# microsoft/M3P

Measured on AMD Instinct MI355X. Metric: pre-train samples/sec (whole node), 12L/768d seq=128+36, higher is better.
Workload: dtype bf16; 1 GPU; cfg2: 12L/768d/12h, 36 regions + 128 tokens, V=250002, 19 MLM targets/seq + ITM BCE, dropout 0.10, adam_inverse_sqrt + clip 5; per_gpu_batch=256, global_batch=256, seq_len=164, parallelism=dp1, prewarm_steps=36

## Files before the change

### m3p_amd/csrc/gemm.hip

```cpp
#include <mutex>
#include <type_traits>
#include "common.hpp"
#include "../../include/m3p_hip.h"
#include <hip/amd_detail/amd_hip_unsafe_atomics.h>

static int g_variant = 1;
extern "C" void m3p_debug_set_variant(int v) { g_variant = (v == 2 || v == 6) ? v : 1; }

namespace {

constexpr int BK = 64;
constexpr int ROWB = BK * 2;

#define M3P_DSR(dst, addr, off) asm volatile("ds_read_b128 %0, %1 offset:" #off : "=v"(dst) : "v"(addr))
#define M3P_TR(dst, addr, off) asm volatile("ds_read_b64_tr_b16 %0, %1 offset:" #off : "=v"(dst) : "v"(addr))
#define M3P_WAIT_LGKM(N) do { __builtin_amdgcn_sched_barrier(0); asm volatile("s_waitcnt lgkmcnt(" #N ")" ::: "memory"); __builtin_amdgcn_sched_barrier(0); } while (0)
#define M3P_WAIT_VM(N) do { __builtin_amdgcn_sched_barrier(0); asm volatile("s_waitcnt vmcnt(" #N ")" ::: "memory"); __builtin_amdgcn_sched_barrier(0); } while (0)
#define M3P_BAR() do { __builtin_amdgcn_s_barrier(); asm volatile("" ::: "memory"); __builtin_amdgcn_sched_barrier(0); } while (0)

__device__ __forceinline__ int xcd_slot(int nwg) {
  const int per_xcd = nwg >> 3;
  return (blockIdx.x & 7) * per_xcd + (blockIdx.x >> 3);
}
__device__ __forceinline__ int strip_width(int tiles_n, int from, int width) {
// ... 543 lines not shown
    if (O8) w8[j] = (O8 == 2) ? pack8<true>(v, scale8, *amax) : pack8<false>(v, scale8, *amax);
  }
  if (O8) piece8_write(r8, w8, lane);
  bf16* Cp = C + (size_t)mrow0 * ldc + nw + sch * 8;
  if (O8) {
    const uint32_t la = lds_addr(r1), l8 = lds_addr(r8);
    const int row8 = lane >> 2, c8 = lane & 3;
    u32x4_lds Ra, Rb, R8;
    lds_r128(la + ep_off<true>(srow, sch * 16), Ra);
    lds_r128(la + ep_off<true>(8 + srow, sch * 16), Rb);
    lds_r128(l8 + row8 * 64 + (c8 << 4), R8);
    asm volatile("s_waitcnt lgkmcnt(0)" : "+v"(Ra), "+v"(Rb), "+v"(R8));
    st16p<true>(Cp + (size_t)srow * ldc, u32x4{Ra[0], Ra[1], Ra[2], Ra[3]});
    st16p<true>(Cp + (size_t)(8 + srow) * ldc, u32x4{Rb[2], Rb[3], Rb[0], Rb[1]});
    st16p<true>(o8 + (size_t)(mrow0 + row8) * ld8 + nw + ((c8 ^ ((row8 >> 1) & 3)) << 4), u32x4{R8[0], R8[1], R8[2], R8[3]});
    return;
  }
  u32x4 R2[2];
#pragma unroll
  for (int it = 0; it < 2; ++it) {
    const int row = it * 8 + srow;
    R2[it] = flip_halves(*reinterpret_cast<const u32x4*>(r1 + ep_off<true>(row, sch * 16)), it & 1);
  }
#pragma unroll
  for (int it = 0; it < 2; ++it) st16p<true>(Cp + (size_t)(it * 8 + srow) * ldc, R2[it]);
  if (O8) piece8_store(o8, ld8, mrow0, nw, r8, lane);
}

__device__ __forceinline__ void epilogue_half_lse(bf16* __restrict__ C, int ldc, float2* __restrict__ stats, int V, int mrow0, int nw,
                                                  char* r1, const f32x4 (&rows0)[4], const f32x4 (&rows1)[4],
                                                  const f32x4 (&biasv)[4], int lane, bool edge) {
  constexpr float kLog2e = 1.4426950408889634f;
  const int fr = lane & 15, fg = lane >> 4;
  const int srow = lane >> 3, sch = lane & 7;
#pragma unroll
  for (int ii = 0; ii < 2; ++ii) {
    f32x4 x[4];
#pragma unroll
    for (int j = 0; j < 4; ++j) {
      x[j] = (ii ? rows1[j] : rows0[j]) + biasv[j];
      const bf16x4 xb = bf16x4{(bf16)x[j][0], (bf16)x[j][1], (bf16)x[j][2], (bf16)x[j][3]};
      *reinterpret_cast<bf16x4*>(r1 + ep_off8<true>(ii * 16 + fr, (j * 16 + fg * 4) * 2)) = xb;
#pragma unroll
      for (int r = 0; r < 4; ++r) x[j][r] = (float)xb[r];
    }
    if (edge) {
#pragma unroll
      for (int j = 0; j < 4; ++j)
#pragma unroll
        for (int r = 0; r < 4; ++r)
          if (nw + j * 16 + fg * 4 + r >= V) x[j][r] = -INFINITY;
    }
    f32x4 m4 = x[0];
#pragma unroll
    for (int j = 1; j < 4; ++j)
#pragma unroll
      for (int r = 0; r < 4; ++r) m4[r] = fmaxf(m4[r], x[j][r]);
    float m = fmaxf(fmaxf(m4[0], m4[1]), fmaxf(m4[2], m4[3]));
    m = fmaxf(m, __shfl_xor(m, 16, 64));
    m = fmaxf(m, __shfl_xor(m, 32, 64));
    const float mb = (m == -INFINITY) ? 0.f : m * kLog2e;
    f32x4 s4 = f32x4{0.f, 0.f, 0.f, 0.f};
#pragma unroll
    for (int j = 0; j < 4; ++j) {
      const f32x4 a = x[j] * kLog2e - mb;
#pragma unroll
      for (int r = 0; r < 4; ++r) s4[r] += __builtin_amdgcn_exp2f(a[r]);
    }
    float sm = (s4[0] + s4[1]) + (s4[2] + s4[3]);
    sm += __shfl_xor(sm, 16, 64);
    sm += __shfl_xor(sm, 32, 64);
    if (fg == 0) stats[mrow0 + ii * 16 + fr] = float2{m, sm};
  }
  bf16* Cp = C + (size_t)mrow0 * ldc + nw + sch * 8;
#pragma unroll
  for (int it = 0; it < 4; ++it) {
    const int row = it * 8 + srow;
    st16p<true>(Cp + (size_t)row * ldc, flip_halves(*reinterpret_cast<const u32x4*>(r1 + ep_off<true>(row, sch * 16)), it & 1));
  }
}

constexpr int M3P_EPI_BIAS_EXP = 11;
struct CeRowRef { float c; int32_t y; };
__device__ __forceinline__ void epilogue_half_exp(bf16* __restrict__ C, int ldc, float* __restrict__ stats, const CeRowRef* __restrict__ ref,
                                                  int V, int mrow0, int nw, char* r1, const f32x4 (&rows0)[4], const f32x4 (&rows1)[4],
                                                  const f32x4 (&biasv)[4], int lane, bool edge) {
  constexpr float kLog2e = 1.4426950408889634f;
  const int fr = lane & 15, fg = lane >> 4;
  const int srow = lane >> 3, sch = lane & 7;
  const float2 rf[2] = {*reinterpret_cast<const float2*>(ref + mrow0 + fr), *reinterpret_cast<const float2*>(ref + mrow0 + 16 + fr)};
#pragma unroll
  for (int ii = 0; ii < 2; ++ii) {
    const float cb = rf[ii].x * kLog2e;
    const int tc = __builtin_bit_cast(int, rf[ii].y) - nw - fg * 4;
    f32x4 x[4];
#pragma unroll
    for (int j = 0; j < 4; ++j) {
      const f32x4 a = ((ii ? rows1[j] : rows0[j]) + biasv[j]) * kLog2e - cb;
#pragma unroll
      for (int r = 0; r < 4; ++r) x[j][r] = __builtin_amdgcn_exp2f(a[r]);
    }
    if (edge) {
#pragma unroll
      for (int j = 0; j < 4; ++j)
#pragma unroll
        for (int r = 0; r < 4; ++r)
          if (nw + j * 16 + fg * 4 + r >= V) x[j][r] = 0.f;
    }
    if (__any((unsigned)(tc + fg * 4) < 64u)) {
#pragma unroll
      for (int j = 0; j < 4; ++j)
#pragma unroll
        for (int r = 0; r < 4; ++r)
          if (j * 16 + r == tc) x[j][r] = 0.f;
    }
    f32x4 s4 = f32x4{0.f, 0.f, 0.f, 0.f};
#pragma unroll
    for (int j = 0; j < 4; ++j) {
      const bf16x4 xb = bf16x4{(bf16)x[j][0], (bf16)x[j][1], (bf16)x[j][2], (bf16)x[j][3]};
      *reinterpret_cast<bf16x4*>(r1 + ep_off8<true>(ii * 16 + fr, (j * 16 + fg * 4) * 2)) = xb;
#pragma unroll
      for (int r = 0; r < 4; ++r) s4[r] += (float)xb[r];
    }
    float sm = (s4[0] + s4[1]) + (s4[2] + s4[3]);
    sm += __shfl_xor(sm, 16, 64);
    sm += __shfl_xor(sm, 32, 64);
    if (fg == 0) stats[mrow0 + ii * 16 + fr] = sm;
  }
  bf16* Cp = C + (size_t)mrow0 * ldc + nw + sch * 8;
#pragma unroll
  for (int it = 0; it < 4; ++it) {
    const int row = it * 8 + srow;
    st16p<true>(Cp + (size_t)row * ldc, flip_halves(*reinterpret_cast<const u32x4*>(r1 + ep_off<true>(row, sch * 16)), it & 1));
  }
}

constexpr int GQ_TAB_LO = 0x3A00, GQ_TAB_HI = 0x4100, GQ_TAB_N = GQ_TAB_HI - GQ_TAB_LO;
constexpr int GQ_TAB_BYTES = GQ_TAB_N * 4;
__device__ __forceinline__ void geluq_table_fill(uint32_t* tab, int tid, int nthreads) {
  for (int i = tid; i < GQ_TAB_N; i += nthreads) {
    const float xm = __builtin_bit_cast(float, ((uint32_t)(GQ_TAB_LO + i) << 16) | 0x8000u);
    const float tail = 0.5f * erfcf(xm * 0.70710678118654752440f);
    const float gd = (1.0f - tail) + xm * 0.39894228040143267794f * __expf(-0.5f * xm * xm);
    tab[i] = (__builtin_bit_cast(uint32_t, tail) & 0xFFFFFF00u) | gelu_grad_code(gd);
  }
}
__device__ __forceinline__ void lds_r32(uint32_t a, uint32_t& v) { asm volatile("ds_read_b32 %0, %1" : "=v"(v) : "v"(a)); }
template <int O8 = 0>
__device__ __forceinline__ void epilogue_piece_geluq_lut(bf16* __restrict__ C, int ldc, uint8_t* __restrict__ qout, int mrow0, int nw,
                                                         char* r1, const f32x4 (&rows)[4], int lane, uint32_t tab_off,
                                                         uint8_t* __restrict__ o8 = nullptr, int ld8 = 0, float scale8 = 1.f, float* amax = nullptr,
                                                         char* r8 = nullptr) {
  const int fr = lane & 15, fg = lane >> 4;
  const int srow = lane >> 3, sch = lane & 7;
  uint32_t w8[4];
  uint32_t w[4][4];
#pragma unroll
  for (int j = 0; j < 4; ++j)
#pragma unroll
    for (int r = 0; r < 4; ++r) {
      const float xf = rows[j][r];
      const uint32_t xb = __builtin_bit_cast(uint32_t, xf);
      const uint32_t mag = __builtin_amdgcn_ubfe(xb, 16, 15);
      const uint32_t idx = min(max(mag, (uint32_t)GQ_TAB_LO), (uint32_t)(GQ_TAB_HI - 1));
      lds_r32((idx << 2) + tab_off, w[j][r]);
    }
  asm volatile("s_waitcnt lgkmcnt(0)" : "+v"(w[0][0]), "+v"(w[0][1]), "+v"(w[0][2]), "+v"(w[0][3]), "+v"(w[1][0]), "+v"(w[1][1]), "+v"(w[1][2]), "+v"(w[1][3]),
                                        "+v"(w[2][0]), "+v"(w[2][1]), "+v"(w[2][2]), "+v"(w[2][3]), "+v"(w[3][0]), "+v"(w[3][1]), "+v"(w[3][2]), "+v"(w[3][3]));
  const uint32_t la = lds_addr(r1);
  u32x4 code;
#pragma unroll
  for (int j = 0; j < 4; ++j) {
    f32x4 hv;
    float xs[4];
#pragma unroll
    for (int r = 0; r < 4; ++r) {
      xs[r] = rows[j][r];
      float mx;
      asm("v_max_f32 %0, 0, %1" : "=v"(mx) : "v"(xs[r]));
      asm("v_fma_f32 %0, -|%1|, %2, %3" : "=v"(hv[r]) : "v"(xs[r]), "v"(w[j][r]), "v"(mx));
    }
    const uint32_t x0 = __builtin_bit_cast(uint32_t, xs[0]), x1 = __builtin_bit_cast(uint32_t, xs[1]);
    const uint32_t x2 = __builtin_bit_cast(uint32_t, xs[2]), x3 = __builtin_bit_cast(uint32_t, xs[3]);
    const uint32_t blo = __builtin_amdgcn_perm(w[j][1], w[j][0], 0x0c0c0400u), bhi = __builtin_amdgcn_perm(w[j][3], w[j][2], 0x04000c0cu);
    const uint32_t slo = __builtin_amdgcn_perm(x1, x0, 0x0c0c0b09u), shi = __builtin_amdgcn_perm(x3, x2, 0x0b090c0cu);
    code[j] = (blo | bhi) ^ (slo | shi);
    lds_w64(la + ep_off8<true>(fr, (j * 16 + fg * 4) * 2), bf16x4{(bf16)hv[0], (bf16)hv[1], (bf16)hv[2], (bf16)hv[3]});
    if (O8) w8[j] = pack8<false>(hv, scale8, *amax);
  }
  st16p<true>(qout + lane * 16, code);
  if (O8) piece8_write(r8, w8, lane);
  u32x4 R[2];
  u32x4_lds R8;
  lds_r128(la + ep_off<true>(srow, sch * 16), R[0]);
  lds_r128(la + ep_off<true>(8 + srow, sch * 16), R[1]);
  const int row8 = lane >> 2, c8 = lane & 3;
  if (O8) {
    lds_r128(lds_addr(r8) + row8 * 64 + (c8 << 4), R8);
    asm volatile("s_waitcnt lgkmcnt(0)" : "+v"(R[0]), "+v"(R[1]), "+v"(R8));
  } else {
    asm volatile("s_waitcnt lgkmcnt(0)" : "+v"(R[0]), "+v"(R[1]));
  }
  bf16* Cp = C + (size_t)mrow0 * ldc + nw + sch * 8;
  st16p<true>(Cp + (size_t)srow * ldc, R[0]);
  st16p<true>(Cp + (size_t)(8 + srow) * ldc, flip_halves(R[1], true));
  if (O8) st16p<true>(o8 + (size_t)(mrow0 + row8) * ld8 + nw + ((c8 ^ ((row8 >> 1) & 3)) << 4), u32x4{R8[0], R8[1], R8[2], R8[3]});
}


template <int EPI>
// ... 152 lines not shown
        u32x4 auxt0[4], auxt1[4];
        load_aux_rows_issue<EPI>(ep, mw, nw, lane, auxt0);
        load_aux_rows_issue<EPI>(ep, mw + 32, nw, lane, auxt1);
        auto do_half = [&](const int hf, const u32x4 (&auxt)[4]) {
          f32x4 rows[2][4];
#pragma unroll
          for (int ii = 0; ii < 2; ++ii)
#pragma unroll
            for (int j = 0; j < 4; ++j) rows[ii][j] = acc[2 * hf + ii][j];
          f32x4 biasv[4];
          bf16x4 auxv[2][4];
          load_bias4<EPI>(ep, nw, lane, biasv);
          load_aux_rows_finish<EPI>(lane, r1, auxt, auxv);
          epilogue_half<EPI>(ep, C, ldc, N, mw + 32 * hf, nw, r1, rows, biasv, auxv, lane, csum, gtab);
        };
        do_half(0, auxt0);
        do_half(1, auxt1);
      } else {
#pragma unroll
        for (int i = 0; i < 4; ++i)
#pragma unroll
          for (int j = 0; j < 4; ++j)
            epilogue_store<EPI>(ep, C, ldc, M, N, mw + i * 16 + fr, nw + j * 16 + fg * 4, acc[i][j], csum[j]);
      }
#pragma unroll
      for (int i = 0; i < 4; ++i)
#pragma unroll
        for (int j = 0; j < 4; ++j) acc[i][j] = f32x4{0.f, 0.f, 0.f, 0.f};
      if (step + 1 < total) {
        M3P_WAIT_LGKM(0);
        __builtin_amdgcn_s_barrier();
        asm volatile("" ::: "memory");
      }
    }
    cur = nxt;
  }
  if ((EPI == M3P_EPI_DGELU || EPI == M3P_EPI_MUL) && ep.colsum && csum_nw >= 0) flush_csum();
}


template <class T>
__device__ __forceinline__ const T* uniform_ptr(const T* p) {
  const uint64_t v = reinterpret_cast<uint64_t>(p);
  const uint32_t lo = __builtin_amdgcn_readfirstlane((uint32_t)v), hi = __builtin_amdgcn_readfirstlane((uint32_t)(v >> 32));
  return reinterpret_cast<const T*>(((uint64_t)hi << 32) | lo);
}

template <int EPI, bool DYN = false, bool O8 = false>
__global__ __launch_bounds__(512)
void gemm_nt_w8_kernel(const bf16* __restrict__ A, int lda, const bf16* __restrict__ W, int ldw,
                       bf16* __restrict__ C, int ldc, int M, int N, int K, M3PEpilogue ep,
                       int tiles_m, int tiles_n, int* __restrict__ tile_ctr) {
  constexpr int BM = 256, BN = 256, NWAVES = 8;
  constexpr int A_BYTES = BM * ROWB, STAGE = (BM + BN) * ROWB;
  extern __shared__ __attribute__((aligned(16))) char smem[];

  const int tid = threadIdx.x, lane = tid & 63;
  const int wid = __builtin_amdgcn_readfirstlane(tid >> 6);
  const int ntiles = tiles_m * tiles_n;
  const int strip_w = strip_width(tiles_n, 9, 4);
  auto split_tile = [&](int t, int& tm, int& tn) {
    const int strip = t / (tiles_m * strip_w);
    const int rem = t - strip * tiles_m * strip_w;
    const int bn = min(strip_w, tiles_n - strip * strip_w);
    tm = rem / bn;
    tn = strip * strip_w + (rem - tm * bn);
  };
  const int nwg = gridDim.x;
  const int per_xcd = nwg >> 3;
  const int xcd = blockIdx.x & 7;
  const int slot = xcd_slot(nwg);
  if (slot >= ntiles) return;
  const int nk = K / BK;
  constexpr bool dyn = DYN;
  auto tile_of = [&](int q) { return q * nwg + slot; };
  const int my_tiles = (ntiles - slot + nwg - 1) / nwg;
  const int total = my_tiles * nk;
  int t_ld = slot, t_cmp = slot, t_next = -1;
  int pop_state = 0;
  unsigned popped = 0;
  constexpr bool kMulE = (EPI == M3P_EPI_DGELU || EPI == M3P_EPI_MUL || EPI == M3P_EPI_MULQ);
  constexpr bool kAuxE = (EPI == M3P_EPI_BIAS_DROP_RES || EPI == M3P_EPI_RES || kMulE);
  constexpr bool kGqLut = (EPI == M3P_EPI_BIAS_GELUQ);
  constexpr int kTabBytes = (EPI == M3P_EPI_DGELU) ? GELU_TAB_N * (int)sizeof(float) : (kGqLut ? GQ_TAB_BYTES : 0);
  float* gtab = (EPI == M3P_EPI_DGELU) ? reinterpret_cast<float*>(smem + 2 * STAGE) : nullptr;
  if (EPI == M3P_EPI_DGELU) gelu_grad_table_fill(gtab, tid, 512);
  if (kGqLut) geluq_table_fill(reinterpret_cast<uint32_t*>(smem + 2 * STAGE), tid, 512);
  int* const mbox = reinterpret_cast<int*>(smem + 2 * STAGE + kTabBytes);

  const int sr = lane >> 3, sc = (lane & 7) ^ sr;
  int l_kt = 0, l_q = 0;
  bool l_alive = true;
  __amdgpu_buffer_rsrc_t a_rsrc, w_rsrc;
  auto set_load_tile = [&](int t) {
    int tm, tn;
    split_tile(t, tm, tn);
    const bf16* a_src = A + (size_t)(tm * BM + wid * 32) * lda;
    const bf16* w_src = W + (size_t)(tn * BN + wid * 32) * ldw;
    a_rsrc = __builtin_amdgcn_make_buffer_rsrc(const_cast<bf16*>(uniform_ptr(a_src)), 0, 0xffffffff, 0x00020000);
    w_rsrc = __builtin_amdgcn_make_buffer_rsrc(const_cast<bf16*>(uniform_ptr(w_src)), 0, 0xffffffff, 0x00020000);
  };
  const uint32_t a_lane = (uint32_t)(sr * lda + sc * 8) * 2u, w_lane = (uint32_t)(sr * ldw + sc * 8) * 2u;
  auto issue_load = [&](int s, int piece) {
    char* sa = smem + s * STAGE;
    const int k0 = l_kt * BK;
    const int pc = piece & 3;
    char* base = sa + (piece < 4 ? 0 : A_BYTES) + wid * 4096;
    const uint32_t soff = __builtin_amdgcn_readfirstlane((uint32_t)k0 * 2u + (uint32_t)pc * (uint32_t)((piece < 4 ? lda : ldw) * 16) - (uint32_t)pc * 1024u);
#define W8_LDB(IMM) __builtin_amdgcn_raw_ptr_buffer_load_lds(piece < 4 ? a_rsrc : w_rsrc, LDS_PTR(base), 16, piece < 4 ? a_lane : w_lane, soff, IMM, 0)
    switch (pc) {
      case 0: W8_LDB(0); break;
      case 1: W8_LDB(1024); break;
      case 2: W8_LDB(2048); break;
      default: W8_LDB(3072); break;
    }
#undef W8_LDB
  };
  auto load_done = [&]() {
    if constexpr (!dyn) {
      if (++l_kt == nk) { l_kt = 0; ++l_q; if (l_q < my_tiles) set_load_tile(tile_of(l_q)); }
    } else {
      ++l_kt;
      if (l_kt == 3) {
        pop_state = 1;
        if (wid == 0 && lane == 0) popped = __hip_atomic_fetch_add(reinterpret_cast<unsigned*>(tile_ctr) + xcd, 1u, __ATOMIC_RELAXED, __HIP_MEMORY_SCOPE_AGENT);
      }
      if (l_kt == nk) {
        l_kt = 0;
        t_ld = t_next;
        t_next = -1;
        if (t_ld >= 0) set_load_tile(t_ld); else l_alive = false;
      }
    }
  };
  auto stage_next = [&](int s) {
#pragma unroll
    for (int pc = 0; pc < 8; ++pc) issue_load(s, pc);
    load_done();
  };

  const int wm = wid >> 2, wn = wid & 3;
  const int fr = lane & 15, fg = lane >> 4;
  const uint32_t lds0 = (uint32_t)(uintptr_t)(__attribute__((address_space(3))) char*)smem;
  uint32_t a_addr[2], b_addr[2];
#pragma unroll
  for (int ks = 0; ks < 2; ++ks) {
    const int ch = ((fg + 4 * ks) ^ (fr & 7)) * 16;
    a_addr[ks] = lds0 + (wm * 128 + fr) * ROWB + ch;
    b_addr[ks] = lds0 + A_BYTES + (wn * 64 + fr) * ROWB + ch;
  }
  auto read_w = [&](uint32_t ba, bf16x8 (&wf)[4]) {
    M3P_DSR(wf[0], ba, 0); M3P_DSR(wf[1], ba, 2048); M3P_DSR(wf[2], ba, 4096); M3P_DSR(wf[3], ba, 6144);
  };
  auto read_a_lo = [&](uint32_t aa, bf16x8 (&af)[4]) {
    M3P_DSR(af[0], aa, 0); M3P_DSR(af[1], aa, 2048); M3P_DSR(af[2], aa, 4096); M3P_DSR(af[3], aa, 6144);
  };
  auto read_a_hi = [&](uint32_t aa, bf16x8 (&af)[4]) {
    M3P_DSR(af[0], aa, 8192); M3P_DSR(af[1], aa, 10240); M3P_DSR(af[2], aa, 12288); M3P_DSR(af[3], aa, 14336);
  };

  f32x4 acc[8][4];
#pragma unroll
  for (int i = 0; i < 8; ++i)
#pragma unroll
    for (int j = 0; j < 4; ++j) acc[i][j] = f32x4{0.f, 0.f, 0.f, 0.f};
  if constexpr (kGqLut) {
    int tm0, tn0;
    split_tile(slot, tm0, tn0);
    const float* bp = ep.bias + tn0 * BN + wn * 64 + fg * 4;
#pragma unroll
    for (int j = 0; j < 4; ++j) {
      const f32x4 b = *reinterpret_cast<const f32x4*>(bp + j * 16);
#pragma unroll
      for (int i = 0; i < 8; ++i) acc[i][j] = b;
    }
  }
  auto mfma_q = [&](auto half_c, const bf16x8 (&af)[4], const bf16x8 (&wf)[4]) {
    constexpr int I0 = 4 * decltype(half_c)::value;
    __builtin_amdgcn_s_setprio(1);
#pragma unroll
    for (int i = 0; i < 4; ++i)
#pragma unroll
      for (int j = 0; j < 4; ++j)
        acc[I0 + i][j] = __builtin_amdgcn_mfma_f32_16x16x32_bf16(wf[j], af[i], acc[I0 + i][j], 0, 0, 0);
    __builtin_amdgcn_s_setprio(0);
  };
  using H0 = std::integral_constant<int, 0>;
  using H1 = std::integral_constant<int, 1>;

  set_load_tile(slot);
  stage_next(0);
#define W8_H1 (dyn ? h1d : (step + 1 < total))
#define W8_MORE2 (dyn ? l_alive : more2)
  bool h1d = l_alive;
  if (dyn ? h1d : (total > 1)) {
    stage_next(1);
    asm volatile("s_waitcnt vmcnt(8)" ::: "memory");
  } else {
    asm volatile("s_waitcnt vmcnt(0)" ::: "memory");
  }
  __builtin_amdgcn_s_barrier();
  asm volatile("" ::: "memory");

  bf16x8 fa0[4], fa1[4], fw0[4], fw1[4];
  read_w(b_addr[0], fw0);
  read_a_lo(a_addr[0], fa0);
  M3P_WAIT_LGKM(0);
  int c_kt = 0, c_q = 0;
  const bool io_aligned = ((ldc & 7) == 0) && (((uintptr_t)C & 15) == 0) &&
                          (!(EPI == M3P_EPI_BIAS_GELU) || (((ep.ld_out2 & 7) == 0) && (((uintptr_t)ep.out2 & 15) == 0))) &&
                          (!ep.bias || (((uintptr_t)ep.bias & 15) == 0)) &&
                          (!ep.aux || (((ep.ld_aux & 7) == 0) && (((uintptr_t)ep.aux & 15) == 0)));
  f32x4 csum[4];
#pragma unroll
  for (int j = 0; j < 4; ++j) csum[j] = f32x4{0.f, 0.f, 0.f, 0.f};
  int csum_nw = -1;
  auto flush_csum = [&]() {
#pragma unroll
    for (int j = 0; j < 4; ++j)
#pragma unroll
      for (int r = 0; r < 4; ++r) {
        float sfl = csum[j][r];
        sfl += __shfl_xor(sfl, 1, 64); sfl += __shfl_xor(sfl, 2, 64);
        sfl += __shfl_xor(sfl, 4, 64); sfl += __shfl_xor(sfl, 8, 64);
        const int n = csum_nw + j * 16 + fg * 4 + r;
        if (fr == 0 && n < N) unsafeAtomicAdd(ep.colsum + n, sfl);
        csum[j][r] = 0.f;
      }
  };
  float amax_run = 0.f;
  if constexpr (O8 && EPI == M3P_EPI_MULQ) reinterpret_cast<float*>(smem + 2 * STAGE + 8 * 2048)[tid] = 0.f;
  bool spread_pending = false;
  for (int step = 0; dyn || step < total; ++step) {
    const int cur = step & 1, nxt = cur ^ 1;
    const bool last_kt = (c_kt + 1 == nk);
    const bool more2 = dyn ? false : (step + 2 < total);
    const uint32_t so = cur * STAGE;
    const bool pend = spread_pending;
    if (pend) { issue_load(nxt, 3); issue_load(nxt, 4); issue_load(nxt, 5); }
    read_a_hi(a_addr[0] + so, fa1);
    __builtin_amdgcn_sched_barrier(0);
    mfma_q(H0{}, fa0, fw0);
    M3P_WAIT_LGKM(0);
    if (pend) { issue_load(nxt, 6); issue_load(nxt, 7); }
    read_w(b_addr[1] + so, fw1);
    read_a_lo(a_addr[1] + so, fa0);
    __builtin_amdgcn_sched_barrier(0);
    mfma_q(H1{}, fa1, fw0);
    if (pend) { load_done(); spread_pending = false; }
    M3P_WAIT_LGKM(0);
    read_a_hi(a_addr[1] + so, fa1);
    __builtin_amdgcn_sched_barrier(0);
    mfma_q(H0{}, fa0, fw1);
    M3P_WAIT_LGKM(0);
    asm volatile("s_waitcnt vmcnt(0)" ::: "memory");
    __builtin_amdgcn_s_barrier();
    asm volatile("" ::: "memory");
    __builtin_amdgcn_sched_barrier(0);
    if (dyn && pop_state) {
      if (pop_state == 1) {
        if (wid == 0 && lane == 0) {
          const int p = per_xcd + (int)popped, q = p / per_xcd;
          const int t = q * nwg + xcd * per_xcd + (p - q * per_xcd);
          *mbox = (t < ntiles) ? t : -1;
        }
        pop_state = 2;
      } else {
        t_next = __builtin_amdgcn_readfirstlane(*mbox);
        pop_state = 0;
      }
      __builtin_amdgcn_sched_barrier(0);
    }
    const bool req = W8_MORE2 && (!last_kt || !kAuxE);
    if (req) {
      issue_load(cur, 0); issue_load(cur, 1); issue_load(cur, 2);
      spread_pending = true;
    }
    if (W8_H1 && !last_kt) {
      read_w(b_addr[0] + nxt * STAGE, fw0);
      read_a_lo(a_addr[0] + nxt * STAGE, fa0);
    }
    __builtin_amdgcn_sched_barrier(0);
    mfma_q(H1{}, fa1, fw1);
    M3P_WAIT_LGKM(0);

    if (++c_kt == nk) {
      c_kt = 0;
      const int t = dyn ? t_cmp : tile_of(c_q);
      if (dyn) t_cmp = t_ld; else ++c_q;
      int tm, tn;
      split_tile(t, tm, tn);
      const int m0 = tm * BM, n0 = tn * BN;
      const int mw = m0 + wm * 128, nw = n0 + wn * 64;
      if (kMulE && ep.colsum && csum_nw != nw) {
        if (csum_nw >= 0) flush_csum();
        csum_nw = nw;
      }
      const bool fast = io_aligned && (m0 + BM <= M) && (n0 + BN <= N);
      if constexpr (EPI == M3P_EPI_BIAS_LSE || EPI == M3P_EPI_BIAS_EXP) {
        if (fast) {
          char* r1 = smem + 2 * STAGE + wid * 4096;
          f32x4 biasv[4];
#pragma unroll
          for (int j = 0; j < 4; ++j) biasv[j] = *reinterpret_cast<const f32x4*>(ep.bias + nw + j * 16 + (lane >> 4) * 4);
          const int V = ep.ld_out2;
          const bool edge = (nw + 64 > V);
          if constexpr (EPI == M3P_EPI_BIAS_EXP) {
            float* st = reinterpret_cast<float*>(ep.out2) + (size_t)(tn * 4 + wn) * M;
            const CeRowRef* ref = reinterpret_cast<const CeRowRef*>(ep.row_ref);
#pragma unroll
            for (int hf = 0; hf < 4; ++hf) {
              epilogue_half_exp(C, ldc, st, ref, V, mw + 32 * hf, nw, r1, acc[2 * hf], acc[2 * hf + 1], biasv, lane, edge);
              __builtin_amdgcn_sched_barrier(0);
            }
          } else {
            float2* st = reinterpret_cast<float2*>(ep.out2) + (size_t)(tn * 4 + wn) * M;
#pragma unroll
            for (int hf = 0; hf < 4; ++hf) {
              epilogue_half_lse(C, ldc, st, V, mw + 32 * hf, nw, r1, acc[2 * hf], acc[2 * hf + 1], biasv, lane, edge);
              __builtin_amdgcn_sched_barrier(0);
            }
          }
        }
      } else if constexpr (kGqLut) {
        f32x4 bnext[4];
        {
          const bool more_tiles = dyn ? (t_cmp >= 0) : (c_q < my_tiles);
          int tm2 = tm, tn2 = tn;
          if (more_tiles) split_tile(dyn ? t_cmp : tile_of(c_q), tm2, tn2);
          const float* bp = ep.bias + tn2 * BN + wn * 64 + fg * 4;
#pragma unroll
          for (int j = 0; j < 4; ++j) bnext[j] = *reinterpret_cast<const f32x4*>(bp + j * 16);
        }
        {
          char* r1 = smem + 2 * STAGE + kTabBytes + wid * 2048;
          const uint32_t tab_off = lds0 + 2 * STAGE - 4 * GQ_TAB_LO;
          uint8_t* qo = reinterpret_cast<uint8_t*>(ep.out2) + gq_block_offset(tm, tn, tiles_n, wid, 0);
          if constexpr (O8) {
            const float sc8 = ep.scale8 ? *ep.scale8 : 1.f;
#pragma unroll
            for (int hp = 0; hp < 8; ++hp) {
              epilogue_piece_geluq_lut<1>(C, ldc, qo + 1024 * hp, mw + 16 * hp, nw, r1, acc[hp], lane, tab_off,
                                          reinterpret_cast<uint8_t*>(ep.out8), ep.ld_out8, sc8, &amax_run,
                                          smem + 2 * STAGE + kTabBytes + 8 * 2048 + wid * 1024);
              __builtin_amdgcn_sched_barrier(0);
            }
          } else {
#pragma unroll
            for (int hp = 0; hp < 8; ++hp) {
              epilogue_piece_geluq_lut(C, ldc, qo + 1024 * hp, mw + 16 * hp, nw, r1, acc[hp], lane, tab_off);
              __builtin_amdgcn_sched_barrier(0);
            }
          }
        }
#pragma unroll
        for (int i = 0; i < 8; ++i)
#pragma unroll
          for (int j = 0; j < 4; ++j) acc[i][j] = bnext[j];
      } else if constexpr (EPI == M3P_EPI_MULQ) {
        if (fast) {
          const uint8_t* qp = reinterpret_cast<const uint8_t*>(ep.aux) + gq_block_offset(tm, tn, tiles_n, wid, 0) + lane * 16;
          char* r1 = smem + 2 * STAGE + wid * 2048;
#define MQ_LD(off) (*reinterpret_cast<const u32x4*>(qp + (off)))
          u32x4 qa = MQ_LD(0), qb = MQ_LD(1024);
          __builtin_amdgcn_sched_barrier(0);
          if (W8_MORE2) { issue_load(cur, 0); issue_load(cur, 1); issue_load(cur, 2); spread_pending = true; }
          __builtin_amdgcn_sched_barrier(0);
          if constexpr (O8) {
            const float sc8 = ep.scale8 ? *ep.scale8 : 1.f;
            uint8_t* o8 = reinterpret_cast<uint8_t*>(ep.out8);
            float* amax_slot = reinterpret_cast<float*>(smem + 2 * STAGE + 8 * 2048) + tid;
            float amax_t = *amax_slot;
#pragma unroll
            for (int hp = 0; hp < 8; ++hp) {
              u32x4 qc = qb;
              if (hp + 2 < 8) qc = MQ_LD((hp + 2) * 1024);
              char* r8 = smem + 2 * STAGE + 8 * 2048 + 2048 + wid * 1024;
              epilogue_pieceq<2>(C, ldc, mw + 16 * hp, nw, r1, acc[hp], qa, lane, csum, o8, ep.ld_out8, sc8, &amax_t, r8);
              __builtin_amdgcn_sched_barrier(0);
              qa = qb; qb = qc;
            }
            *amax_slot = amax_t;
          } else {
#pragma unroll
          for (int hp = 0; hp < 8; hp += 2) {
            u32x4 qc = qa, qd = qb;
            if (hp + 2 < 8) qc = MQ_LD((hp + 2) * 1024);
            epilogue_pieceq(C, ldc, mw + 16 * hp, nw, r1, acc[hp], qa, lane, csum);
            __builtin_amdgcn_sched_barrier(0);
            if (hp + 3 < 8) qd = MQ_LD((hp + 3) * 1024);
            epilogue_pieceq(C, ldc, mw + 16 * (hp + 1), nw, r1, acc[hp + 1], qb, lane, csum);
            __builtin_amdgcn_sched_barrier(0);
            qa = qc; qb = qd;
          }
          }
#undef MQ_LD
        }
      } else if (fast && kMulE) {
        char* r1 = smem + 2 * STAGE + kTabBytes + wid * 2048;
        u32x4 ta[2], tb[2];
        aux16_issue(ep, mw, nw, lane, ta);
        __builtin_amdgcn_sched_barrier(0);
        if (W8_MORE2) { issue_load(cur, 0); issue_load(cur, 1); issue_load(cur, 2); spread_pending = true; }
        __builtin_amdgcn_sched_barrier(0);
#pragma unroll
        for (int hp = 0; hp < 8; hp += 2) {
          aux16_issue(ep, mw + 16 * (hp + 1), nw, lane, tb);
          epilogue_piece16<EPI>(ep, C, ldc, mw + 16 * hp, nw, r1, acc[hp], ta, lane, csum, gtab);
          __builtin_amdgcn_sched_barrier(0);
          if (hp + 2 < 8) aux16_issue(ep, mw + 16 * (hp + 2), nw, lane, ta);
          epilogue_piece16<EPI>(ep, C, ldc, mw + 16 * (hp + 1), nw, r1, acc[hp + 1], tb, lane, csum, gtab);
          __builtin_amdgcn_sched_barrier(0);
        }
      } else if (fast) {
        char* r1 = smem + 2 * STAGE + wid * 4096;
        f32x4 biasv[4];
        load_bias4<EPI>(ep, nw, lane, biasv);
        u32x4 aux0[4];
        if (kAuxE) {
          load_aux_rows_issue<EPI>(ep, mw, nw, lane, aux0);
          __builtin_amdgcn_sched_barrier(0);
          if (W8_MORE2) { issue_load(cur, 0); issue_load(cur, 1); issue_load(cur, 2); spread_pending = true; }
          __builtin_amdgcn_sched_barrier(0);
        }
#pragma unroll
        for (int hf = 0; hf < 4; ++hf) {
          f32x4 rows[2][4];
#pragma unroll
          for (int ii = 0; ii < 2; ++ii)
#pragma unroll
            for (int j = 0; j < 4; ++j) rows[ii][j] = acc[2 * hf + ii][j];
          bf16x4 auxv[2][4];
          if (kAuxE && hf == 0) load_aux_rows_finish<EPI, true>(lane, r1, aux0, auxv);
          else load_aux_rows<EPI, true>(ep, mw + 32 * hf, nw, lane, r1, auxv);
          epilogue_half<EPI, true>(ep, C, ldc, N, mw + 32 * hf, nw, r1, rows, biasv, auxv, lane, csum, gtab);
          __builtin_amdgcn_sched_barrier(0);
        }
      } else {
        if (kAuxE && W8_MORE2) { issue_load(cur, 0); issue_load(cur, 1); issue_load(cur, 2); spread_pending = true; }
#pragma unroll
        for (int i = 0; i < 8; ++i)
#pragma unroll
          for (int j = 0; j < 4; ++j)
            epilogue_store<EPI>(ep, C, ldc, M, N, mw + i * 16 + fr, nw + j * 16 + fg * 4, acc[i][j], csum[j]);
      }
      if constexpr (!kGqLut) {
#pragma unroll
        for (int i = 0; i < 8; ++i)
#pragma unroll
          for (int j = 0; j < 4; ++j) acc[i][j] = f32x4{0.f, 0.f, 0.f, 0.f};
      }
      if (W8_H1) {
        read_w(b_addr[0] + nxt * STAGE, fw0);
        read_a_lo(a_addr[0] + nxt * STAGE, fa0);
        M3P_WAIT_LGKM(0);
      }
    }
    if (dyn) {
      if (!h1d) break;
      h1d = l_alive;
    }
  }
  if (kMulE && ep.colsum && csum_nw >= 0) flush_csum();
  if constexpr (O8 && (EPI == M3P_EPI_BIAS_GELUQ || EPI == M3P_EPI_MULQ)) {
    if (ep.amax8) {
      float* wmax = reinterpret_cast<float*>(smem + 2 * STAGE + kTabBytes);
      if constexpr (EPI == M3P_EPI_MULQ) amax_run = reinterpret_cast<float*>(smem + 2 * STAGE + 8 * 2048)[tid];
      const float mxw = wave_max(amax_run);
      __syncthreads();
      if (lane == 0) wmax[wid] = mxw;
      __syncthreads();
      if (tid == 0) {
        float mx = wmax[0];
#pragma unroll
        for (int w = 1; w < NWAVES; ++w) mx = fmaxf(mx, wmax[w]);
        unsigned int* slot = reinterpret_cast<unsigned int*>(ep.amax8);
        if (__float_as_uint(mx) > __builtin_nontemporal_load(slot)) atomicMax(slot, __float_as_uint(mx));
      }
    }
  }
#undef W8_H1
#undef W8_MORE2
}

typedef __attribute__((ext_vector_type(8))) int i32x8;
typedef __attribute__((ext_vector_type(4))) int i32x4;
template <int EPI, bool A_BF8>
__global__ __launch_bounds__(512)
void gemm_nt_w8f8_kernel(const uint8_t* __restrict__ A, int lda, const uint8_t* __restrict__ W, int ldw,
                         bf16* __restrict__ C, int ldc, int M, int N, int K, M3PEpilogue ep,
                         int tiles_m, int tiles_n) {
  constexpr int BM = 256, BN = 256, NWAVES = 8, BK8 = 128;
  constexpr int A_BYTES = BM * ROWB, STAGE = (BM + BN) * ROWB;
  extern __shared__ __attribute__((aligned(16))) char smem[];

  const int tid = threadIdx.x, lane = tid & 63;
  const int wid = __builtin_amdgcn_readfirstlane(tid >> 6);
  const int ntiles = tiles_m * tiles_n;
  const int strip_w = strip_width(tiles_n, 12, 4);
  const int nwg = gridDim.x;
  const int slot = xcd_slot(nwg);
  auto tile_of = [&](int q) { return q * nwg + slot; };
  const int my_tiles = (ntiles > slot) ? (ntiles - slot + nwg - 1) / nwg : 0;
  if (my_tiles == 0) return;
  constexpr bool kMulE = (EPI == M3P_EPI_DGELU || EPI == M3P_EPI_MUL);
  constexpr bool kAuxE = (EPI == M3P_EPI_BIAS_DROP_RES || EPI == M3P_EPI_RES || kMulE);
  constexpr bool kGqLut = (EPI == M3P_EPI_BIAS_GELUQ);
  constexpr int kTabBytes = (EPI == M3P_EPI_DGELU) ? GELU_TAB_N * (int)sizeof(float) : (kGqLut ? GQ_TAB_BYTES : 0);
  float* gtab = (EPI == M3P_EPI_DGELU) ? reinterpret_cast<float*>(smem + 2 * STAGE) : nullptr;
  if (EPI == M3P_EPI_DGELU) gelu_grad_table_fill(gtab, tid, 512);
  if (kGqLut) geluq_table_fill(reinterpret_cast<uint32_t*>(smem + 2 * STAGE), tid, 512);
  const int nk = K / BK8;
  const int total = my_tiles * nk;
  const float dsc = (ep.descale_a ? *ep.descale_a : 1.f) * (ep.descale_b ? *ep.descale_b : 1.f);

  const int sr = lane >> 3, sc = (lane & 7) ^ sr;
  const uint8_t* a_src;
  const uint8_t* w_src;
  const size_t a_step = (size_t)64 * lda, w_step = (size_t)64 * ldw;
  int l_q = 0, l_kt = 0;
  auto set_load_tile = [&](int q) {
    int tm, tn;
    split_tile(tile_of(q), tiles_m, tiles_n, strip_w, tm, tn);
    a_src = A + (size_t)(tm * BM + wid * 8 + sr) * lda + sc * 16;
    w_src = W + (size_t)(tn * BN + wid * 8 + sr) * ldw + sc * 16;
  };
  auto issue_load = [&](int s, int piece) {
    char* sa = smem + s * STAGE;
    const int k0 = l_kt * BK8;
// ... 541 lines not shown
    return M3P_KERN_NT_W4;
  if (M >= 1024) return M3P_KERN_NT_RING;
  return M3P_KERN_NT_128;
}

template <int EPI>
int launch_nt(const bf16* A, int lda, const bf16* W, int ldw, bf16* C, int ldc, int M, int N, int K,
              const M3PEpilogue& ep, hipStream_t st) {
  int want_queue = 0;
  const int plan = nt_plan(EPI, M, N, K, &want_queue);
  if (plan == M3P_KERN_NT_SKINNY) {
    if constexpr (EPI != M3P_EPI_DGELU && EPI != M3P_EPI_MUL) {
      if (M <= 16) return launch_nt_skinny<EPI, 1>(A, lda, W, ldw, C, ldc, M, N, K, ep, st);
      if (M <= 32) return launch_nt_skinny<EPI, 2>(A, lda, W, ldw, C, ldc, M, N, K, ep, st);
      if (M <= 64) return launch_nt_skinny<EPI, 4>(A, lda, W, ldw, C, ldc, M, N, K, ep, st);
      return launch_nt_skinny<EPI, 8>(A, lda, W, ldw, C, ldc, M, N, K, ep, st);
    }
  }
  if (plan == M3P_KERN_NT_W8) {
    const int tiles_m = M / 256, tiles_n = N / 256;
    const size_t lds = 2 * 512 * ROWB + (EPI == M3P_EPI_DGELU ? GELU_TAB_N * sizeof(float) : 0) +
                       ((EPI == M3P_EPI_DGELU || EPI == M3P_EPI_MUL) ? 8 * 2048 : 8 * 4096);
    constexpr auto kern = gemm_nt_w8_kernel<EPI>;
    if (int rc = set_max_lds<kern>(lds)) return rc;
    const int grid = persistent_grid(tiles_m * tiles_n);
    constexpr bool kQueueOk = !(EPI == M3P_EPI_DGELU || EPI == M3P_EPI_MUL);
    int* ctr = nullptr;
    if (kQueueOk && want_queue) {
      hipError_t e;
      ctr = tq_acquire(st, &e);
      if (e != hipSuccess) return (int)e;
    }
    if constexpr (kQueueOk) if (ctr) {
      constexpr auto kern_d = gemm_nt_w8_kernel<EPI, true>;
      if (int rc = set_max_lds<kern_d>(lds)) return rc;
      hipLaunchKernelGGL(kern_d, dim3(grid), dim3(512), lds, st, A, lda, W, ldw, C, ldc, M, N, K, ep, tiles_m, tiles_n, ctr);
      M3P_CHECK_LAUNCH();
      return M3P_OK;
    }
    hipLaunchKernelGGL(kern, dim3(grid), dim3(512), lds, st, A, lda, W, ldw, C, ldc, M, N, K, ep, tiles_m, tiles_n, ctr);
    M3P_CHECK_LAUNCH();
    return M3P_OK;
  }
  if (plan == M3P_KERN_NT_W4) {
    constexpr int BM = 256, BN = 256;
    const int tiles_m = (M + BM - 1) / BM, tiles_n = (N + BN - 1) / BN;
    const size_t lds = 2 * (BM + BN) * 128 + 4 * EP_HALF;
    const bool rows = (EPI == M3P_EPI_BIAS_DROP_RES && ep.rng_rows != nullptr);
    constexpr auto kern_rows = gemm_nt_w4_kernel<(EPI == M3P_EPI_BIAS_DROP_RES ? M3P_EPI_DROP_RES_ROWS : EPI)>, kern_plain = gemm_nt_w4_kernel<EPI>;
    if (int rc = rows ? set_max_lds<kern_rows>(lds) : set_max_lds<kern_plain>(lds)) return rc;
    auto kern = rows ? kern_rows : kern_plain;
    const int grid = persistent_grid(tiles_m * tiles_n);
    const long long wbytes = 2LL * N * K, abytes = 2LL * M * K;
    const int m_fast = (wbytes > (64LL << 20) && abytes < wbytes) ? 1 : 0;
    hipLaunchKernelGGL(kern, dim3(grid), dim3(256), lds, st, A, lda, W, ldw, C, ldc, M, N, K, ep, tiles_m, tiles_n, m_fast);
    M3P_CHECK_LAUNCH();
    return M3P_OK;
  }
  if (plan == M3P_KERN_NT_RING) {
    constexpr int BM = 256, BN = 128;
    const int tiles_m = (M + BM - 1) / BM, tiles_n = (N + BN - 1) / BN;
    const size_t lds = 3 * (BM + BN) * ROWB + (EPI == M3P_EPI_DGELU ? GELU_TAB_N * sizeof(float) : 0);
    constexpr auto kern = gemm_nt_ring_kernel<EPI>;
    if (int rc = set_max_lds<kern>(lds)) return rc;
    const int grid = persistent_grid(tiles_m * tiles_n);
    hipLaunchKernelGGL(kern, dim3(grid), dim3(512), lds, st, A, lda, W, ldw, C, ldc, M, N, K, ep, tiles_m, tiles_n);
    M3P_CHECK_LAUNCH();
    return M3P_OK;
  }
  constexpr int BM = 128, BN = 128;
  const int tiles_m = (M + BM - 1) / BM, tiles_n = (N + BN - 1) / BN;
  const size_t lds = 2 * (BM + BN) * ROWB;
  constexpr auto kern = gemm_nt_kernel<BM, BN, EPI>;
  if (int rc = set_max_lds<kern>(lds)) return rc;
  hipLaunchKernelGGL(kern, dim3(tiles_m * tiles_n), dim3(256), lds, st, A, lda, W, ldw, C, ldc, M, N, K, ep,
                     tiles_m, tiles_n);
  M3P_CHECK_LAUNCH();
  return M3P_OK;
}

template <int EPI>
static int launch_nt_gq(const bf16* A, int lda, const bf16* W, int ldw, bf16* C, int ldc, int M, int N, int K,
                        const M3PEpilogue& ep, hipStream_t st) {
  if (M < 1024 || (M % 256) || (N % 256) || N < 512 || (K % 64) || (lda % 8) || (ldw % 8) || (ldc % 8) || ((uintptr_t)C & 15))
    return M3P_EINVAL;
  if (EPI == M3P_EPI_MULQ && (!ep.aux || ((uintptr_t)ep.aux & 15))) return M3P_EINVAL;
  constexpr bool kLse = (EPI == M3P_EPI_BIAS_LSE || EPI == M3P_EPI_BIAS_EXP);
  if ((EPI == M3P_EPI_BIAS_GELUQ || kLse) && (!ep.out2 || ((uintptr_t)ep.out2 & 15) || !ep.bias || ((uintptr_t)ep.bias & 15)))
    return M3P_EINVAL;
  if (kLse && (ep.ld_out2 <= 0 || ep.ld_out2 > N)) return M3P_EINVAL;
  if (EPI == M3P_EPI_BIAS_EXP && (!ep.row_ref || ((uintptr_t)ep.row_ref & 7))) return M3P_EINVAL;
  const int tiles_m = M / 256, tiles_n = N / 256;
  const size_t lds = 2 * 512 * ROWB + ((EPI == M3P_EPI_BIAS_GELUQ) ? GQ_TAB_BYTES + 8 * 2048 + 8 * 1024 : 8 * (EPI != M3P_EPI_MULQ ? 4096 : 2048)) +
                     (EPI == M3P_EPI_MULQ ? 2048 + 8 * 1024 : 0);
  const int grid = persistent_grid(tiles_m * tiles_n);
  if constexpr (EPI == M3P_EPI_BIAS_GELUQ || EPI == M3P_EPI_MULQ) {
    if (ep.out8) {
      if (((uintptr_t)ep.out8 & 15) || (ep.ld_out8 & 15) || ep.ld_out8 < N || !ep.scale8 || !ep.amax8) return M3P_EINVAL;
      if ((EPI == M3P_EPI_MULQ) != (ep.out8_bf8 != 0)) return M3P_EINVAL;
      constexpr auto kern8 = gemm_nt_w8_kernel<EPI, false, true>;
      if (int rc = set_max_lds<kern8>(lds)) return rc;
      hipLaunchKernelGGL(kern8, dim3(grid), dim3(512), lds, st, A, lda, W, ldw, C, ldc, M, N, K, ep, tiles_m, tiles_n, (int*)nullptr);
      M3P_CHECK_LAUNCH();
      return M3P_OK;
    }
  }
  constexpr auto kern = gemm_nt_w8_kernel<EPI>;
  if (int rc = set_max_lds<kern>(lds)) return rc;
  hipLaunchKernelGGL(kern, dim3(grid), dim3(512), lds, st, A, lda, W, ldw, C, ldc, M, N, K, ep, tiles_m, tiles_n, (int*)nullptr);
  M3P_CHECK_LAUNCH();
  return M3P_OK;
}

constexpr int WG_T = 128;
constexpr int WG_ROWB = WG_T * 2;
constexpr int WG_TILE_BYTES = BK * WG_ROWB;

__device__ __forceinline__ bf16x4 lds_tr16(const char* p) {
  s16x4 v = __builtin_amdgcn_ds_read_tr16_b64_v4i16((__attribute__((address_space(3))) s16x4*)(p));
  return __builtin_bit_cast(bf16x4, v);
}

__global__ __launch_bounds__(256)
void gemm_wgrad_kernel(const bf16* __restrict__ dY, int lddy, const bf16* __restrict__ X, int ldx,
                       float* __restrict__ dW, int lddw, int M, int N, int K, float alpha,
                       int tiles_i, int tiles_j, int m_chunk) {
  extern __shared__ __attribute__((aligned(16))) char smem[];
  const int tid = threadIdx.x, lane = tid & 63;
  const int wid = __builtin_amdgcn_readfirstlane(tid >> 6);
  const int ntile = tiles_i * tiles_j;
  const int id = xcd_remap(blockIdx.x, gridDim.x);
  const int split = id / ntile, tile = id - split * ntile;
  const int ti = tile / tiles_j, tj = tile - ti * tiles_j;
  const int i0 = ti * WG_T, j0 = tj * WG_T;
  const int m_begin = split * m_chunk;
  const int m_end = min(M, m_begin + m_chunk);
  if (m_begin >= m_end) return;

  const int sr = lane >> 4, sc = lane & 15;
  const int n_chunks = (N + 7) / 8, k_chunks = (K + 7) / 8;
  int ycol[4], xcol[4];
#pragma unroll
  for (int i = 0; i < 4; ++i) {
    const int rb = wid + i * 4;
    const int f = sr | (((rb >> 1) & 1) << 2);
    const int gc = sc ^ (f << 1);
    ycol[i] = min(i0 / 8 + gc, n_chunks - 1) * 8;
    xcol[i] = min(j0 / 8 + gc, k_chunks - 1) * 8;
  }

  auto stage = [&](int mt, int s) {
    char* sy = smem + s * 2 * WG_TILE_BYTES;
    char* sx = sy + WG_TILE_BYTES;
    const int mbase = m_begin + mt * BK;
    const bool fullt = (mbase + BK <= m_end);
#pragma unroll
    for (int i = 0; i < 4; ++i) {
      const int rb = wid + i * 4;
      const int m = mbase + rb * 4 + sr;
      if (fullt) {
        __builtin_amdgcn_global_load_lds(GLB_PTR(dY + (size_t)m * lddy + ycol[i]), LDS_PTR(sy + rb * 1024), 16, 0, 0);
        __builtin_amdgcn_global_load_lds(GLB_PTR(X + (size_t)m * ldx + xcol[i]), LDS_PTR(sx + rb * 1024), 16, 0, 0);
      } else {
        uint4 vy = make_uint4(0, 0, 0, 0), vx = make_uint4(0, 0, 0, 0);
        if (m < m_end) {
          vy = *reinterpret_cast<const uint4*>(dY + (size_t)m * lddy + ycol[i]);
          vx = *reinterpret_cast<const uint4*>(X + (size_t)m * ldx + xcol[i]);
// ... 589 lines not shown
```

Baseline: 8246 sequences/s.

## Fold bias into accumulator init and sum exp rows via MFMA in CE epilogue

```diff
diff --git a/m3p_amd/csrc/gemm.hip b/m3p_amd/csrc/gemm.hip
--- a/m3p_amd/csrc/gemm.hip
+++ b/m3p_amd/csrc/gemm.hip
@@ -649,21 +649,20 @@
 
 constexpr int M3P_EPI_BIAS_EXP = 11;
 struct CeRowRef { float c; int32_t y; };
-__device__ __forceinline__ void epilogue_half_exp(bf16* __restrict__ C, int ldc, float* __restrict__ stats, const CeRowRef* __restrict__ ref,
+__device__ __forceinline__ void epilogue_half_exp(bf16* __restrict__ C, int ldc, float* __restrict__ stats, const float2 (&rf)[2],
                                                   int V, int mrow0, int nw, char* r1, const f32x4 (&rows0)[4], const f32x4 (&rows1)[4],
-                                                  const f32x4 (&biasv)[4], int lane, bool edge) {
+                                                  int lane, bool edge) {
   constexpr float kLog2e = 1.4426950408889634f;
   const int fr = lane & 15, fg = lane >> 4;
   const int srow = lane >> 3, sch = lane & 7;
-  const float2 rf[2] = {*reinterpret_cast<const float2*>(ref + mrow0 + fr), *reinterpret_cast<const float2*>(ref + mrow0 + 16 + fr)};
 #pragma unroll
   for (int ii = 0; ii < 2; ++ii) {
-    const float cb = rf[ii].x * kLog2e;
+    const float ncb = -(rf[ii].x * kLog2e);
     const int tc = __builtin_bit_cast(int, rf[ii].y) - nw - fg * 4;
     f32x4 x[4];
 #pragma unroll
     for (int j = 0; j < 4; ++j) {
-      const f32x4 a = ((ii ? rows1[j] : rows0[j]) + biasv[j]) * kLog2e - cb;
+      const f32x4 a = (ii ? rows1[j] : rows0[j]) * kLog2e + ncb;
 #pragma unroll
       for (int r = 0; r < 4; ++r) x[j][r] = __builtin_amdgcn_exp2f(a[r]);
     }
@@ -681,18 +680,20 @@
         for (int r = 0; r < 4; ++r)
           if (j * 16 + r == tc) x[j][r] = 0.f;
     }
-    f32x4 s4 = f32x4{0.f, 0.f, 0.f, 0.f};
-#pragma unroll
-    for (int j = 0; j < 4; ++j) {
-      const bf16x4 xb = bf16x4{(bf16)x[j][0], (bf16)x[j][1], (bf16)x[j][2], (bf16)x[j][3]};
-      *reinterpret_cast<bf16x4*>(r1 + ep_off8<true>(ii * 16 + fr, (j * 16 + fg * 4) * 2)) = xb;
-#pragma unroll
-      for (int r = 0; r < 4; ++r) s4[r] += (float)xb[r];
-    }
-    float sm = (s4[0] + s4[1]) + (s4[2] + s4[3]);
-    sm += __shfl_xor(sm, 16, 64);
-    sm += __shfl_xor(sm, 32, 64);
-    if (fg == 0) stats[mrow0 + ii * 16 + fr] = sm;
+#pragma unroll
+    for (int j = 0; j < 4; ++j)
+      *reinterpret_cast<bf16x4*>(r1 + ep_off8<true>(ii * 16 + fr, (j * 16 + fg * 4) * 2)) =
+          bf16x4{(bf16)x[j][0], (bf16)x[j][1], (bf16)x[j][2], (bf16)x[j][3]};
+  }
+  const bf16 one = (bf16)1.0f;
+  const bf16x8 ones = bf16x8{one, one, one, one, one, one, one, one};
+#pragma unroll
+  for (int ii = 0; ii < 2; ++ii) {
+    const bf16x8 lo = *reinterpret_cast<const bf16x8*>(r1 + ep_off<true>(ii * 16 + fr, fg * 16));
+    const bf16x8 hi = *reinterpret_cast<const bf16x8*>(r1 + ep_off<true>(ii * 16 + fr, (fg + 4) * 16));
+    f32x4 sm = __builtin_amdgcn_mfma_f32_16x16x32_bf16(ones, lo, f32x4{0.f, 0.f, 0.f, 0.f}, 0, 0, 0);
+    sm = __builtin_amdgcn_mfma_f32_16x16x32_bf16(ones, hi, sm, 0, 0, 0);
+    if (fg == 0) stats[mrow0 + ii * 16 + fr] = sm[0];
   }
   bf16* Cp = C + (size_t)mrow0 * ldc + nw + sch * 8;
 #pragma unroll
@@ -1011,6 +1012,7 @@
   constexpr bool kMulE = (EPI == M3P_EPI_DGELU || EPI == M3P_EPI_MUL || EPI == M3P_EPI_MULQ);
   constexpr bool kAuxE = (EPI == M3P_EPI_BIAS_DROP_RES || EPI == M3P_EPI_RES || kMulE);
   constexpr bool kGqLut = (EPI == M3P_EPI_BIAS_GELUQ);
+  constexpr bool kBiasAcc = kGqLut || (EPI == M3P_EPI_BIAS_EXP);
   constexpr int kTabBytes = (EPI == M3P_EPI_DGELU) ? GELU_TAB_N * (int)sizeof(float) : (kGqLut ? GQ_TAB_BYTES : 0);
   float* gtab = (EPI == M3P_EPI_DGELU) ? reinterpret_cast<float*>(smem + 2 * STAGE) : nullptr;
   if (EPI == M3P_EPI_DGELU) gelu_grad_table_fill(gtab, tid, 512);
@@ -1093,7 +1095,7 @@
   for (int i = 0; i < 8; ++i)
 #pragma unroll
     for (int j = 0; j < 4; ++j) acc[i][j] = f32x4{0.f, 0.f, 0.f, 0.f};
-  if constexpr (kGqLut) {
+  if constexpr (kBiasAcc) {
     int tm0, tn0;
     split_tile(slot, tm0, tn0);
     const float* bp = ep.bias + tn0 * BN + wn * 64 + fg * 4;
@@ -1200,7 +1202,8 @@
       }
       __builtin_amdgcn_sched_barrier(0);
     }
-    const bool req = W8_MORE2 && (!last_kt || !kAuxE);
+    constexpr bool kRowRefE = (EPI == M3P_EPI_BIAS_EXP);
+    const bool req = W8_MORE2 && (!last_kt || !(kAuxE || kRowRefE));
     if (req) {
       issue_load(cur, 0); issue_load(cur, 1); issue_load(cur, 2);
       spread_pending = true;
@@ -1226,7 +1229,40 @@
         csum_nw = nw;
       }
       const bool fast = io_aligned && (m0 + BM <= M) && (n0 + BN <= N);
-      if constexpr (EPI == M3P_EPI_BIAS_LSE || EPI == M3P_EPI_BIAS_EXP) {
+      if constexpr (EPI == M3P_EPI_BIAS_EXP) {
+        f32x4 bnext[4];
+        float2 rowref[8];
+        {
+          const CeRowRef* rp = reinterpret_cast<const CeRowRef*>(ep.row_ref) + mw + fr;
+#pragma unroll
+          for (int i = 0; i < 8; ++i) rowref[i] = *reinterpret_cast<const float2*>(rp + 16 * i);
+          const bool more_tiles = dyn ? (t_cmp >= 0) : (c_q < my_tiles);
+          int tm2 = tm, tn2 = tn;
+          if (more_tiles) split_tile(dyn ? t_cmp : tile_of(c_q), tm2, tn2);
+          const float* bp = ep.bias + tn2 * BN + wn * 64 + fg * 4;
+#pragma unroll
+          for (int j = 0; j < 4; ++j) bnext[j] = *reinterpret_cast<const f32x4*>(bp + j * 16);
+        }
+        __builtin_amdgcn_sched_barrier(0);
+        if (W8_MORE2) { issue_load(cur, 0); issue_load(cur, 1); issue_load(cur, 2); spread_pending = true; }
+        __builtin_amdgcn_sched_barrier(0);
+        {
+          char* r1 = smem + 2 * STAGE + wid * 4096;
+          const int V = ep.ld_out2;
+          const bool edge = (nw + 64 > V);
+          float* st = reinterpret_cast<float*>(ep.out2) + (size_t)(tn * 4 + wn) * M;
+#pragma unroll
+          for (int hf = 0; hf < 4; ++hf) {
+            const float2 rf[2] = {rowref[2 * hf], rowref[2 * hf + 1]};
+            epilogue_half_exp(C, ldc, st, rf, V, mw + 32 * hf, nw, r1, acc[2 * hf], acc[2 * hf + 1], lane, edge);
+            __builtin_amdgcn_sched_barrier(0);
+          }
+        }
+#pragma unroll
+        for (int i = 0; i < 8; ++i)
+#pragma unroll
+          for (int j = 0; j < 4; ++j) acc[i][j] = bnext[j];
+      } else if constexpr (EPI == M3P_EPI_BIAS_LSE) {
         if (fast) {
           char* r1 = smem + 2 * STAGE + wid * 4096;
           f32x4 biasv[4];
@@ -1234,21 +1270,11 @@
           for (int j = 0; j < 4; ++j) biasv[j] = *reinterpret_cast<const f32x4*>(ep.bias + nw + j * 16 + (lane >> 4) * 4);
           const int V = ep.ld_out2;
           const bool edge = (nw + 64 > V);
-          if constexpr (EPI == M3P_EPI_BIAS_EXP) {
-            float* st = reinterpret_cast<float*>(ep.out2) + (size_t)(tn * 4 + wn) * M;
-            const CeRowRef* ref = reinterpret_cast<const CeRowRef*>(ep.row_ref);
-#pragma unroll
-            for (int hf = 0; hf < 4; ++hf) {
-              epilogue_half_exp(C, ldc, st, ref, V, mw + 32 * hf, nw, r1, acc[2 * hf], acc[2 * hf + 1], biasv, lane, edge);
-              __builtin_amdgcn_sched_barrier(0);
-            }
-          } else {
-            float2* st = reinterpret_cast<float2*>(ep.out2) + (size_t)(tn * 4 + wn) * M;
-#pragma unroll
-            for (int hf = 0; hf < 4; ++hf) {
-              epilogue_half_lse(C, ldc, st, V, mw + 32 * hf, nw, r1, acc[2 * hf], acc[2 * hf + 1], biasv, lane, edge);
-              __builtin_amdgcn_sched_barrier(0);
-            }
+          float2* st = reinterpret_cast<float2*>(ep.out2) + (size_t)(tn * 4 + wn) * M;
+#pragma unroll
+          for (int hf = 0; hf < 4; ++hf) {
+            epilogue_half_lse(C, ldc, st, V, mw + 32 * hf, nw, r1, acc[2 * hf], acc[2 * hf + 1], biasv, lane, edge);
+            __builtin_amdgcn_sched_barrier(0);
           }
         }
       } else if constexpr (kGqLut) {
@@ -1373,7 +1399,7 @@
           for (int j = 0; j < 4; ++j)
             epilogue_store<EPI>(ep, C, ldc, M, N, mw + i * 16 + fr, nw + j * 16 + fg * 4, acc[i][j], csum[j]);
       }
-      if constexpr (!kGqLut) {
+      if constexpr (!kBiasAcc) {
 #pragma unroll
         for (int i = 0; i < 8; ++i)
 #pragma unroll
@@ -2081,7 +2107,8 @@
 template <int EPI>
 static int launch_nt_gq(const bf16* A, int lda, const bf16* W, int ldw, bf16* C, int ldc, int M, int N, int K,
                         const M3PEpilogue& ep, hipStream_t st) {
-  if (M < 1024 || (M % 256) || (N % 256) || N < 512 || (K % 64) || (lda % 8) || (ldw % 8) || (ldc % 8) || ((uintptr_t)C & 15))
+  if (M < (EPI == M3P_EPI_BIAS_EXP ? 256 : 1024) || (M % 256) || (N % 256) || N < 512 || (K % 64) || (lda % 8) || (ldw % 8) || (ldc % 8) ||
+      ((uintptr_t)C & 15))
     return M3P_EINVAL;
   if (EPI == M3P_EPI_MULQ && (!ep.aux || ((uintptr_t)ep.aux & 15))) return M3P_EINVAL;
   constexpr bool kLse = (EPI == M3P_EPI_BIAS_LSE || EPI == M3P_EPI_BIAS_EXP);
```

Result: no change. 8268 sequences/s, median of 6 (+0.3%).
